# PatrickHwang/Explicit-tf2-Recommendation

Measured on AMD Instinct MI355X. Metric: examples/sec fwd+bwd, DeepFM 10M-vocab x16d batch 8192, higher is better.
Workload: dtype f32; 1 GPU; DeepFM fwd+bwd, 26 categorical fields, 10M-vocab x 16d, batch 8192 (BASELINE.json metric); vocab=10000000, fields=26, embedding_dims=16, batch_per_gpu=8192, id_distribution=uniform, parallelism=single GPU, global_batch=8192, hipgraph=one graph per 5 steps, 32 resident batches

## Files before the change

### explicit-tf2-recommendation_amd/csrc/colsort.hip

```cpp
#include "common.h"

namespace {

constexpr uint32_t PADW = 0xFFFFFFFFu;

struct ColSortArgs {
  int64_t B; int F; int64_t V; int key_bits; int pos_bits; int passes; int digit_bits;
  int32_t* perm;
  int64_t* col_uid;
  int32_t* col_seg;
  int32_t* col_nu;
  int* bad;
  int32_t* dloc;
};

constexpr int CS_T = 1024, CS_W = CS_T / 64, CS_DB = 10, CS_BINS = 1 << CS_DB;
constexpr int CS_BKB = 13, CS_NBK = 1 << CS_BKB, CS_BIG = 32, CS_PROBE = 16;
static_assert(CS_BINS == CS_T, "the count scan gives every thread one digit");

#ifdef REC_SORT_STAMPS
__device__ unsigned long long g_sort_stamps[256 * 16];
#define SSTAMP(k) do { if (threadIdx.x == 0) g_sort_stamps[blockIdx.x * 16 + (k)] = wall_clock64(); } while (0)
#else
#define SSTAMP(k) do {} while (0)
#endif

constexpr int SORT_MAX_COLS = 256;
struct SortCols {
  const int64_t* p[SORT_MAX_COLS];
};

static inline void colsort_digits(int key_bits, int* passes, int* digit_bits) {
  const int p = (key_bits + CS_DB - 1) / CS_DB;
  *passes = p;
  *digit_bits = (key_bits + p - 1) / p;
}

template <int KPT>
__global__ __launch_bounds__(CS_T, 4) void colsort_kernel(SortCols cols, const int64_t* __restrict__ col_lo, ColSortArgs a) {
  extern __shared__ __attribute__((aligned(16))) uint32_t sml[];
  constexpr int NW = CS_T * KPT;
  uint32_t* words = sml;
  uint32_t* cnt = sml + NW;
  uint32_t* wtot = cnt + CS_W * CS_BINS;
  const int tid = threadIdx.x, lane = tid & 63, wave = tid >> 6;
  const int f = blockIdx.x;
  const int64_t B = a.B;
  const int64_t lo = col_lo[f];
  const int pb = a.pos_bits;
  const uint32_t pmask = (1u << pb) - 1u;
  uint32_t* wcnt = cnt + wave * CS_BINS;
  const unsigned long long lt = (1ull << lane) - 1ull;
  SSTAMP(0);
  uint32_t w[KPT];
  bool bad = false;
  const int64_t* col = cols.p[f];
#pragma unroll
  for (int r = 0; r < KPT; ++r) {
    const int e = wave * (64 * KPT) + r * 64 + lane;
    w[r] = PADW;
    if (e < B) {
      const int64_t id = col[e];
      int64_t key = id - lo;
      if (key < 0 || key >= (int64_t(1) << a.key_bits) || (uint64_t)id >= (uint64_t)a.V) {
        bad = true;
        key = key < 0 ? 0 : (int64_t(1) << a.key_bits) - 1;
      }
      w[r] = ((uint32_t)key << pb) | (uint32_t)e;
    }
  }
  if (bad && a.bad) *a.bad = 1;
  SSTAMP(1);
  const int wbits = a.key_bits + pb;
  const int bsh = wbits > CS_BKB ? wbits - CS_BKB : 0;
  uint32_t* bk = cnt;
  static_assert(CS_NBK == 8 * CS_T && CS_NBK <= CS_W * CS_BINS, "8 buckets per thread, inside the counters");
#pragma unroll
  for (int i = 0; i < 2; ++i) reinterpret_cast<uint4*>(bk)[i * CS_T + tid] = make_uint4(0u, 0u, 0u, 0u);
  int hot = 0;
#pragma unroll
  for (int r = 0; r < KPT; ++r) {
    const bool real = wave * (64 * KPT) + r * 64 + lane < B;
    const uint32_t b0 = __shfl(w[r] >> bsh, 0, 64);
    hot |= __popcll(__ballot(real && (w[r] >> bsh) == b0)) > CS_PROBE;
  }
  bool fast = !__syncthreads_or(hot);
  if (fast) {
#pragma unroll
    for (int r = 0; r < KPT; ++r)
      if (wave * (64 * KPT) + r * 64 + lane < B) atomicAdd(&bk[w[r] >> bsh], 1u);
    __syncthreads();
    const uint4 q0 = reinterpret_cast<const uint4*>(bk)[2 * tid], q1 = reinterpret_cast<const uint4*>(bk)[2 * tid + 1];
    uint32_t c[8] = {q0.x, q0.y, q0.z, q0.w, q1.x, q1.y, q1.z, q1.w};
    uint32_t run = 0, mx = 0;
#pragma unroll
    for (int q = 0; q < 8; ++q) {
      run += c[q];
      mx = max(mx, c[q]);
    }
    uint32_t incl = run;
#pragma unroll
    for (int o = 1; o < 64; o <<= 1) {
      const uint32_t t = __shfl_up(incl, o, 64);
      if (lane >= o) incl += t;
    }
    if (lane == 63) wtot[wave] = incl;
    __syncthreads();
    uint32_t base = incl - run;
#pragma unroll
    for (int q = 0; q < CS_W; ++q)
      if (q < wave) base += wtot[q];
#pragma unroll
    for (int q = 0; q < 8; ++q) {
      const uint32_t n = c[q];
      c[q] = base;
      base += n;
    }
    reinterpret_cast<uint4*>(bk)[2 * tid] = make_uint4(c[0], c[1], c[2], c[3]);
    reinterpret_cast<uint4*>(bk)[2 * tid + 1] = make_uint4(c[4], c[5], c[6], c[7]);
    fast = !__syncthreads_or(mx > (uint32_t)CS_BIG);
  }
  SSTAMP(2);
  if (fast) {
#pragma unroll
    for (int r = 0; r < KPT; ++r) {
      const int e = wave * (64 * KPT) + r * 64 + lane;
      if (e < B) words[atomicAdd(&bk[w[r] >> bsh], 1u)] = w[r];
      else words[e] = PADW;
    }
    __syncthreads();
    SSTAMP(3);
    uint32_t dst[KPT];
#pragma unroll
    for (int r = 0; r < KPT; ++r) {
      const int e = wave * (64 * KPT) + r * 64 + lane;
      dst[r] = (uint32_t)e;
      if (e < B) {
        const uint32_t b = w[r] >> bsh;
        const uint32_t end = bk[b];
        uint32_t j = b > 0 ? bk[b - 1] : 0u, rk = j;
        for (; j < end; ++j) rk += words[j] < w[r] ? 1u : 0u;
        dst[r] = rk;
      }
    }
    __syncthreads();
#pragma unroll
    for (int r = 0; r < KPT; ++r) words[dst[r]] = w[r];
    __syncthreads();
    SSTAMP(4);
  }
  for (int pass = 0; pass < (fast ? 0 : a.passes); ++pass) {
    const int shift = pb + pass * a.digit_bits;
    const int nb = min(a.digit_bits, a.key_bits - pass * a.digit_bits);
    const uint32_t dmask = (1u << nb) - 1u;
    if (pass > 0) {
#pragma unroll
      for (int r = 0; r < KPT; ++r) w[r] = words[wave * (64 * KPT) + r * 64 + lane];
    }
#pragma unroll
    for (int i = 0; i < CS_BINS / 256; ++i) reinterpret_cast<uint4*>(wcnt)[i * 64 + lane] = make_uint4(0u, 0u, 0u, 0u);
    uint32_t below[KPT];
#pragma unroll
    for (int c0 = 0; c0 < KPT; c0 += 8) {
      unsigned long long m[8];
#pragma unroll
      for (int r = 0; r < 8; ++r) m[r] = ~0ull;
      for (int b = 0; b < nb; ++b) {
#pragma unroll
        for (int r = 0; r < 8; ++r) {
          const uint32_t s = (uint32_t)__builtin_amdgcn_sbfe((int)w[c0 + r], shift + b, 1);
          const unsigned long long bal = __ballot(s != 0u);
          m[r] &= ~(bal ^ (((unsigned long long)s << 32) | s));
        }
      }
      uint32_t old[8];
      int lead[8];
#pragma unroll
      for (int r = 0; r < 8; ++r) {
        lead[r] = __ffsll((long long)m[r]) - 1;
        below[c0 + r] = (uint32_t)__popcll(m[r] & lt);
        old[r] = 0u;
        if (below[c0 + r] == 0u) old[r] = atomicAdd(&wcnt[(w[c0 + r] >> shift) & dmask], (uint32_t)__popcll(m[r]));
      }
#pragma unroll
      for (int r = 0; r < 8; ++r) below[c0 + r] += (uint32_t)__shfl((int)old[r], lead[r], 64);
    }
    __syncthreads();
    {
      uint32_t c[CS_W];
      uint32_t run = 0;
#pragma unroll
      for (int q = 0; q < CS_W; ++q) {
        c[q] = cnt[q * CS_BINS + tid];
        run += c[q];
      }
      uint32_t incl = run;
#pragma unroll
      for (int o = 1; o < 64; o <<= 1) {
        const uint32_t v = __shfl_up(incl, o, 64);
        if (lane >= o) incl += v;
      }
      if (lane == 63) wtot[wave] = incl;
      __syncthreads();
      uint32_t base = incl - run;
#pragma unroll
      for (int q = 0; q < CS_W; ++q)
        if (q < wave) base += wtot[q];
#pragma unroll
      for (int q = 0; q < CS_W; ++q) {
        cnt[q * CS_BINS + tid] = base;
        base += c[q];
      }
    }
    __syncthreads();
#pragma unroll
    for (int r = 0; r < KPT; ++r) words[wcnt[(w[r] >> shift) & dmask] + below[r]] = w[r];
    __syncthreads();
    SSTAMP(2 + pass);
  }
  const int s0 = tid * KPT;
  uint32_t v[KPT];
  bool hd[KPT];
  int heads = 0;
  uint32_t prev = s0 > 0 ? words[s0 - 1] : PADW;
#pragma unroll
  for (int r = 0; r < KPT; ++r) {
    const int sp = s0 + r;
    v[r] = words[sp];
    const uint32_t pk = (r == 0 ? prev : v[r - 1]) >> pb;
    hd[r] = sp < B && (sp == 0 || (v[r] >> pb) != pk);
    heads += hd[r] ? 1 : 0;
  }
  int incl = heads;
#pragma unroll
  for (int o = 1; o < 64; o <<= 1) {
    const int t = __shfl_up(incl, o, 64);
    if (lane >= o) incl += t;
  }
  if (lane == 63) wtot[wave] = (uint32_t)incl;
  __syncthreads();
  int woff = 0, all = 0;
  for (int q = 0; q < CS_W; ++q) {
    const int c = (int)wtot[q];
    if (q < wave) woff += c;
    all += c;
  }
  int rank = woff + incl - heads;
  SSTAMP(7);
  static_assert(2 * sizeof(unsigned short) * NW <= sizeof(uint32_t) * CS_W * CS_BINS, "the staging fits the counters");
  uint32_t* st_uq = words;
  unsigned short* st_sg = reinterpret_cast<unsigned short*>(cnt);
  unsigned short* st_dl = st_sg + NW;
  int32_t* permf = a.perm + (int64_t)f * B;
  if ((B & 7) == 0 && KPT == 8) {
    if (s0 < B) {
      int4 p0 = make_int4((int)(v[0] & pmask), (int)(v[1] & pmask), (int)(v[2] & pmask), (int)(v[3] & pmask));
      int4 p1 = make_int4((int)(v[4 % KPT] & pmask), (int)(v[5 % KPT] & pmask), (int)(v[6 % KPT] & pmask), (int)(v[7 % KPT] & pmask));
      *reinterpret_cast<int4*>(permf + s0) = p0;
      *reinterpret_cast<int4*>(permf + s0 + 4) = p1;
    }
  } else {
#pragma unroll
    for (int r = 0; r < KPT; ++r)
      if (s0 + r < B) permf[s0 + r] = (int32_t)(v[r] & pmask);
  }
#pragma unroll
  for (int r = 0; r < KPT; ++r) {
    const int sp = s0 + r;
    if (sp < B) {
      if (hd[r]) {
        st_uq[rank] = v[r] >> pb;
        st_sg[rank] = (unsigned short)sp;
        ++rank;
      }
      st_dl[v[r] & pmask] = (unsigned short)(hd[r] ? (rank - 1) : ((rank - 1) | 0x8000));
    }
  }
  __syncthreads();
#pragma unroll
  for (int r = 0; r < KPT; ++r) {
    const int i = r * CS_T + tid;
    if (i < B) {
      if (a.dloc) {
        const uint32_t d = st_dl[i];
        a.dloc[(int64_t)f * B + i] = (int32_t)((d & 0x7FFFu) | ((d & 0x8000u) << 16));
      }
      if (i < all) {
        a.col_uid[(int64_t)f * B + i] = lo + (int64_t)st_uq[i];
        a.col_seg[(int64_t)f * (B + 1) + i] = (int32_t)st_sg[i];
      } else {
        a.col_seg[(int64_t)f * (B + 1) + i] = (int32_t)B;
      }
    }
  }
  if (tid == 0) a.col_seg[(int64_t)f * (B + 1) + B] = (int32_t)B;
  if (tid == 0) a.col_nu[f] = all;
  SSTAMP(8);
#ifdef REC_SORT_STAMPS
  asm volatile("s_waitcnt vmcnt(0)" ::: "memory");
  SSTAMP(9);
  if (threadIdx.x == 1023) g_sort_stamps[blockIdx.x * 16 + 10] = wall_clock64();
  if (threadIdx.x == 512) g_sort_stamps[blockIdx.x * 16 + 11] = wall_clock64();
#endif
}

static int colsort_widths(int64_t B, int64_t max_key, int* key_bits, int* pos_bits) {
  if (B <= 0 || max_key < 0) return REC_E_ARG;
  if (B > 16384) return REC_E_UNSUPPORTED;
  int pbits = 1, kbits = 1;
  while ((int64_t(1) << pbits) < B) ++pbits;
  while ((int64_t(1) << kbits) <= max_key) ++kbits;
  if (kbits + pbits > 32) return REC_E_UNSUPPORTED;
  if ((((uint64_t)max_key << pbits) | (uint64_t)(B - 1)) >= 0xFFFFFFFFull) return REC_E_UNSUPPORTED;
  *key_bits = kbits;
  *pos_bits = pbits;
  return REC_OK;
}
}

#ifdef REC_SORT_STAMPS
extern "C" int rec_debug_sort_stamps(unsigned long long* host_out) {
  return (int)hipMemcpyFromSymbol(host_out, HIP_SYMBOL(g_sort_stamps), sizeof(unsigned long long) * 256 * 16);
}
#endif
extern "C" size_t rec_colsort_workspace_bytes(int64_t B, int F) {
  if (B <= 0 || F <= 0) return 0;
  return 256;
}

extern "C" int rec_colsort_digits(int64_t B, int64_t max_key, int* passes, int* digit_bits) {
  if (!passes || !digit_bits) return REC_E_ARG;
  int key_bits = 0, pos_bits = 0;
  const int rc = colsort_widths(B, max_key, &key_bits, &pos_bits);
  if (rc != REC_OK) return rc;
  colsort_digits(key_bits, passes, digit_bits);
  return REC_OK;
}

static int colsort_plan(const int64_t* const* cols_host, int F, int64_t B, int64_t V, const int64_t* col_lo,
                        int64_t max_key, int32_t* perm, int64_t* col_uid, int32_t* col_seg, int32_t* col_nu,
                        int32_t* dloc, int* bad_flag, void* workspace, void* stream) {
  if (!cols_host || !col_lo || !perm || !col_uid || !col_seg || !col_nu || !workspace || F <= 0 || B <= 0 || V <= 0 ||
      max_key < 0)
    return REC_E_ARG;
  if (F > SORT_MAX_COLS) return REC_E_UNSUPPORTED;
  int key_bits = 0, pos_bits = 0;
  const int rc = colsort_widths(B, max_key, &key_bits, &pos_bits);
  if (rc != REC_OK) return rc;
  int passes = 0, digit_bits = 0;
  colsort_digits(key_bits, &passes, &digit_bits);
  SortCols cp;
  for (int f = 0; f < F; ++f) {
    if (!cols_host[f]) return REC_E_ARG;
    cp.p[f] = cols_host[f];
  }
  ColSortArgs a{B, F, V, key_bits, pos_bits, passes, digit_bits, perm, col_uid, col_seg, col_nu, bad_flag, dloc};
  hipStream_t st = as_stream(stream);
  const int kpt = B <= 8192 ? 8 : 16;
  const size_t lds = sizeof(uint32_t) * ((size_t)CS_T * kpt + CS_W * CS_BINS + CS_W);
  const hipError_t e = kpt == 8 ? rec_allow_lds<colsort_kernel<8>>(lds) : rec_allow_lds<colsort_kernel<16>>(lds);
  if (e != hipSuccess) return (int)e;
  if (kpt == 8)
    hipLaunchKernelGGL(colsort_kernel<8>, dim3(F), dim3(CS_T), lds, st, cp, col_lo, a);
  else
    hipLaunchKernelGGL(colsort_kernel<16>, dim3(F), dim3(CS_T), lds, st, cp, col_lo, a);
  REC_LAUNCH_CHECK();
  return REC_OK;
}

extern "C" int rec_colsort_plan_i64(const int64_t* const* cols_host, int F, int64_t B, int64_t V, const int64_t* col_lo,
                                    int64_t max_key, int32_t* perm, int64_t* col_uid, int32_t* col_seg, int32_t* col_nu,
                                    int* bad_flag, void* workspace, void* stream) {
  return colsort_plan(cols_host, F, B, V, col_lo, max_key, perm, col_uid, col_seg, col_nu, nullptr, bad_flag, workspace,
                      stream);
}

extern "C" int rec_colsort_plan_dest_i64(const int64_t* const* cols_host, int F, int64_t B, int64_t V,
                                         const int64_t* col_lo, int64_t max_key, int32_t* perm, int64_t* col_uid,
                                         int32_t* col_seg, int32_t* col_nu, int32_t* dloc, int* bad_flag, void* workspace,
                                         void* stream) {
  if (!dloc) return REC_E_ARG;
  return colsort_plan(cols_host, F, B, V, col_lo, max_key, perm, col_uid, col_seg, col_nu, dloc, bad_flag, workspace,
                      stream);
}
```

### include/mi355rec.h

```cpp
#ifndef MI355REC_H
#define MI355REC_H

#include <stdint.h>
#include <stddef.h>

#ifdef __cplusplus
extern "C" {
#endif

#define REC_OK 0
#define REC_E_ARG (-1)
#define REC_E_UNSUPPORTED (-2)
#define REC_E_WORKSPACE (-3)

#define REC_MAX_COLS 128

#define REC_AFM_MAX_F 64
#define REC_AFM_MAX_E 64
#define REC_AFM_MAX_A 16
#define REC_AUTOINT_MAX_F 64
#define REC_AUTOINT_MAX_E 64
#define REC_FIBINET_MAX_F 32
#define REC_FIBINET_MAX_E 64
#define REC_FIBINET_MAX_C 64
#define REC_CIN_MAX_F 64
#define REC_CIN_MAX_E 64
#define REC_CIN_MAX_L 8
#define REC_CIN_MAX_H 256
#define REC_FIELD_CONV_MAX_F 64
#define REC_FIELD_CONV_MAX_E 64
#define REC_FIELD_CONV_MAX_L 3
#define REC_FIELD_CONV_MAX_C 16
#define REC_FIELD_CONV_MAX_KW 8
#define REC_FIELD_CONV_BWD_GRID 1024
#define REC_FGCNN_MAX_PW 8
#define REC_MASKNET_MAX_F 64
#define REC_MASKNET_MAX_E 64
#define REC_MASKNET_MAX_D 512
#define REC_MASKNET_MAX_P 512
#define REC_MASKNET_MAX_O 128
#define REC_MASKNET_MAX_R 4

enum { REC_ACT_NONE = 0, REC_ACT_RELU = 1, REC_ACT_SIGMOID = 2, REC_ACT_TANH = 3 };

enum {
  REC_EPI_NONE = 0,
  REC_EPI_BIAS = 1,
  REC_EPI_BIAS_RELU = 2,
  REC_EPI_BIAS_SIGMOID = 3,
  REC_EPI_BIAS_TANH = 4,
  REC_EPI_CROSS = 5,
  REC_EPI_ADD = 6
};

int rec_version(void);

int rec_index_pack_i64(const int64_t* const* cols_host, int F, int64_t rows, int64_t* X, int64_t ldx,
                       int64_t col0, void* stream);

int rec_block_copy(const void* const* srcs_host, int n, int64_t bytes_each, void* out, void* stream);
int rec_auc_hist_update_f32(const float* prob, const float* label, int64_t n, const float* thresholds, int n_thresholds,
                            int64_t* hist, const float* loss_steps, int n_steps, double* loss_acc, void* stream);

int rec_emb_gather_f32(const float* table, int64_t V, int E, int64_t ld, const int64_t* idx, int64_t n,
                       float* out, int* oob_flag, void* stream);

int rec_emb_fm_fwd_f32(const float* embed, int64_t ld_e, const float* w, int64_t ld_w, const float* bias,
                       int64_t V, int E, const int64_t* idx, int64_t B, int F, float* z, float* prob,
                       float* emb_out, float* sumvec, int* oob_flag, void* stream);

int rec_emb_fm_bwd_vals_f32(const float* embed, int64_t ld_e, int64_t V, int E, const int64_t* idx, int64_t B,
                            int F, const float* gz, const float* sumvec, const float* emb_rows,
                            const float* extra, float* dvals, void* stream);

size_t rec_dedup_workspace_bytes(int64_t n);
int rec_dedup_plan_i64(const int64_t* ids, int64_t n, int64_t V, int64_t* uniq_ids, int32_t* seg_start,
                       int32_t* perm, int64_t* n_uniq, void* workspace, size_t workspace_bytes,
                       void* stream);
int rec_dedup_plan_sorted_lists_i64(const int64_t* ids, int64_t n, const int64_t* list_counts, int n_lists,
                                    int64_t V, int64_t* uniq_ids, int32_t* seg_start, int32_t* perm,
                                    int64_t* n_uniq, void* workspace, size_t workspace_bytes, void* stream);
size_t rec_segment_sum_workspace_bytes(int64_t n, int E);
int rec_segment_sum_f32(const float* vals, int E, const int32_t* perm, const int32_t* seg_start, int64_t n,
                        int32_t row_div, float* out, float* workspace, void* stream);

int rec_gemm_f32(int transA, int transB, int64_t M, int64_t N, int64_t K, const float* A, int64_t lda,
                 const float* B, int64_t ldb, float* C, int64_t ldc, int epilogue, const float* bias,
                 const float* e0, int64_t lde0, const float* e1, int64_t lde1, int split_k,
                 float* workspace, float* aux, void* stream);

int rec_crossnet_mat_bwd_elem_f32(const float* g, const float* x0, const float* u, float* h, float* gx0,
                                  int accumulate, int64_t n, void* stream);

int rec_act_fwd_f32(int act, const float* x, const float* x2, float* y, int64_t n, void* stream);
int rec_act_bwd_f32(int act, const float* post, const float* dpost, float* dpre, int64_t n, void* stream);
size_t rec_colsum_workspace_bytes(int64_t M, int64_t N);
int rec_colsum_f32(const float* X, int64_t M, int64_t N, int64_t ldx, float* out, float* workspace, void* stream);
int rec_colsum_fused_f32(const float* X, int64_t M, int64_t N, int64_t ldx, float* out, float* workspace, int* counters,
                         void* stream);
int rec_axpby_f32(float a, const float* x, float b, float* y, int64_t n, void* stream);
int rec_copy_cols_f32(const float* src, int64_t lds, float* dst, int64_t ldd, int64_t rows, int64_t w,
                      void* stream);

int rec_crossnet_vec_fwd_f32(const float* x0, int64_t B, int D, int L, const float* w, const float* b,
                             float* y, float* xs, void* stream);
size_t rec_crossnet_vec_bwd_workspace_bytes(int64_t B, int D, int L);
int rec_crossnet_vec_bwd_f32(const float* x0, int64_t B, int D, int L, const float* w, const float* xs,
                             const float* gy, float* gx0, float* dw, float* db, void* workspace,
                             void* stream);

int rec_cosine_fwd_f32(const float* u, const float* i, int64_t B, int d, float* out, void* stream);
int rec_cosine_bwd_f32(const float* u, const float* i, int64_t B, int d, const float* gout, float* gu,
                       float* gi, void* stream);

int rec_bce_fwd_bwd_f32(const float* y, const float* p, int64_t n, float* loss, float* dp, float* dz,
                        void* stream);

int rec_adam_dense_f32(float* var, float* m, float* v, const float* g, int64_t n, int64_t t, float lr,
                       float b1, float b2, float eps, void* stream);
float rec_adam_lr_t_f32(float lr, float b1, float b2, int64_t t);
int rec_adam_dense_multi_f32(int n_tensors, float* const* var, float* const* m, float* const* v, const float* const* g,
                             const int64_t* numel, const float* lr_t_dev, float b1, float b2, float eps, void* stream);
int rec_adam_sparse_keras_f32(float* var, int64_t ld, float* m, float* v, int64_t V, int E,
                              const int64_t* uniq_ids, const float* g_rows, const int64_t* n_uniq, int64_t cap,
                              float* side, int64_t t, float lr, float b1, float b2, float eps, void* stream);
int rec_adam_sparse_keras_pair_f32(float* fused, int64_t ld, float* m_e, float* v_e, float* m_w, float* v_w, int64_t V,
                                   int E, const int64_t* uniq_ids, const float* g_e_rows, const float* g_w_rows,
                                   const int64_t* n_uniq, int64_t cap, float* side_e, float* side_w, int64_t t,
                                   float lr, float b1, float b2, float eps, void* stream);

int rec_adam_rows_f32(float* var, int64_t ld, float* m, float* v, int64_t V, int E, const int64_t* uniq_ids,
                      const float* g_rows, const int64_t* n_uniq, int64_t cap, int64_t t, float lr,
                      float b1, float b2, float eps, void* stream);

size_t rec_l2_rows_workspace_bytes(int64_t n, int E);
int rec_l2_rows_f32(const float* table, int64_t ld, int64_t V, int E, const int64_t* uniq_ids, const int64_t* n_uniq,
                    int64_t n, float factor, float* rows_out, float* loss, float* workspace, void* stream);

int rec_l2_normalize_rows_f32(const float* x, int64_t n, int d, int64_t ld_in, float* y, int64_t ld_out, void* stream);
size_t rec_topk_l2_workspace_bytes(int64_t nq, int64_t n, int k);
int rec_topk_l2_f32(const float* queries, int64_t nq, int d, int64_t ldq, const float* items, int64_t n, int64_t ldi,
                    int k, int64_t* out_idx, float* out_dist, void* workspace, size_t workspace_bytes, void* stream);

size_t rec_shard_bucketize_workspace_bytes(int64_t n, int n_shard);
int rec_shard_bucketize_i64(const int64_t* ids, int64_t n, int64_t rows_per_shard, int n_shard,
                            int64_t* perm, int64_t* send_counts, int64_t* local_ids, int* oob_flag,
                            void* workspace, size_t workspace_bytes, void* stream);
int rec_colsort_shard_map_i64(const int32_t* perm, const int64_t* col_uid, const int32_t* col_seg,
                              const int32_t* col_nu, int64_t B, int F, int64_t rows_per_shard, int n_shard,
                              int64_t* uid_local, int64_t* uidx, int64_t* send_counts, int64_t* n_uniq,
                              int* oob_flag, void* stream);
int rec_colsort_shard_map_fixed_i64(const int32_t* perm, const int64_t* col_uid, const int32_t* col_seg,
                                    const int32_t* col_nu, int64_t B, int F, int64_t rows_per_shard, int n_shard,
                                    int64_t cap, int64_t* msg, int64_t* uidx, int32_t* slot_map, int64_t* n_uniq,
                                    int* oob_flag, void* stream);
int rec_shard_slab_map_uslot_i64(const int64_t* uniq_ids, const int64_t* n_uniq, const int32_t* seg_start,
                                 const int32_t* perm, int64_t n, int64_t rows_per_shard, int n_shard, int64_t cap,
                                 int64_t* msg, int64_t* slot, int64_t* uslot, int* oob_flag, void* stream);
int rec_emb_gather_lists_f32(const float* table, int64_t V, int E, int64_t ld, const int64_t* msg, int n_lists,
                             int64_t cap, float* out, int* oob_flag, void* stream);
int rec_dedup_plan_sorted_slabs_i64(const int64_t* msg, int n_lists, int64_t cap, int64_t V, int64_t* uniq_ids,
                                    int32_t* seg_start, int32_t* perm, int64_t* n_uniq, void* workspace,
                                    size_t workspace_bytes, void* stream);
int rec_permute_rows_f32(const float* in, const int64_t* perm, int64_t n, int E, int scatter, float* out,
                         void* stream);

size_t rec_deepfm_fused_workspace_bytes(int64_t B, int F);

size_t rec_colsort_workspace_bytes(int64_t B, int F);
int rec_colsort_digits(int64_t B, int64_t max_key, int* passes, int* digit_bits);
int rec_colsort_plan_i64(const int64_t* const* cols_host, int F, int64_t B, int64_t V, const int64_t* col_lo,
                         int64_t max_key, int32_t* perm, int64_t* col_uid, int32_t* col_seg, int32_t* col_nu,
                         int* bad_flag, void* workspace, void* stream);
int rec_colsort_plan_dest_i64(const int64_t* const* cols_host, int F, int64_t B, int64_t V, const int64_t* col_lo,
                              int64_t max_key, int32_t* perm, int64_t* col_uid, int32_t* col_seg, int32_t* col_nu,
                              int32_t* dloc, int* bad_flag, void* workspace, void* stream);

int rec_deepfm_k0t_f32(const float* K0, int F, float* K0T, void* stream);
int rec_deepfm_fused3_main_f32(const float* table, int64_t ld, int64_t V, const int64_t* const* cols_host, int F,
                               int64_t B, const float* const* weights, const float* label, float* gz, float* vals,
                               float* prob, int* oob_flag, void* workspace, const int32_t* dloc, const int32_t* col_nu,
                               float* g_embed_rows, int64_t* step_dev, const float* lr_table, int64_t n_table,
                               float* lr_t_dev, void* stream);

typedef struct rec_deepfm_lazy_adam {
  float* table; int64_t ld, V;
  float *m_e, *v_e, *m_w, *v_w; int64_t ld_state, ld_wstate;
  const float* lr_t_dev; float b1, b2, eps;
  int32_t* last; const int64_t* step_dev;
} rec_deepfm_lazy_adam;
int rec_deepfm_fused_post_f32(int F, int64_t B, const float* gz, const float* vals, float* const* grads, float* loss,
                              void* workspace, const int32_t* perm, const int64_t* col_uid, const int32_t* col_seg,
                              const int32_t* col_nu, int64_t* uniq_ids, float* g_embed_rows, float* g_w_rows,
                              int64_t* n_uniq, const int32_t* slot_map, int direct, const rec_deepfm_lazy_adam* adam,
                              void* stream);
int rec_adam_keras_catchup_f32(const int64_t* col_uid, const int32_t* col_nu, int64_t B, int F, float* table, int64_t ld,
                               int64_t V, float* m_e, float* v_e, int64_t ld_state, float* m_w, float* v_w,
                               int64_t ld_wstate, const int32_t* last, const int64_t* step_dev, const float* lr_table,
                               int64_t n_table, float b1, float b2, float eps, void* stream);
int rec_adam_keras_flush_f32(float* table, int64_t ld, int64_t V, float* m_e, float* v_e, int64_t ld_state, float* m_w,
                             float* v_w, int64_t ld_wstate, int32_t* last, const int64_t* step_dev, const float* lr_table,
                             int64_t n_table, float b1, float b2, float eps, void* stream);

size_t rec_dssm_fused_workspace_bytes(int64_t B, int E, int F_u, int F_i);
int rec_dssm_fused_main_f32(const float* u_table, int64_t u_ld, int64_t u_V, const int64_t* u_ids, int F_u,
                            const float* i_table, int64_t i_ld, int64_t i_V, const int64_t* i_ids, int F_i, int E,
                            int h1, int h2, int d_out, int64_t B, const float* const* weights, const float* label,
                            float* u_vals, float* i_vals, float* user_emb, float* item_emb, float* score, int* oob_flag,
                            void* workspace, size_t workspace_bytes, int64_t* step_dev, const float* lr_table,
                            int64_t n_table, float* lr_t_dev, void* stream);
int rec_dssm_fused_post_f32(int64_t B, int E, int F_u, int F_i, const void* workspace, size_t workspace_bytes,
                            float* const* grads, float* loss, const float* u_vals, const int32_t* u_perm,
                            const int32_t* u_seg, const int64_t* u_uniq, const int64_t* u_n_uniq, float* u_rows,
                            const float* i_vals, const int32_t* i_perm, const int32_t* i_seg, const int64_t* i_uniq,
                            const int64_t* i_n_uniq, float* i_rows, float* const* adam, int64_t u_ld, int64_t u_V,
                            int64_t i_ld, int64_t i_V, const float* lr_t_dev, float b1, float b2, float eps,
                            void* stream);

enum { REC_DACT_NONE = 0, REC_DACT_RELU = 1, REC_DACT_SIGMOID = 2, REC_DACT_TANH = 3,
       REC_DACT_DICE = 4,
       REC_DACT_PRELU = 5 };
int rec_din_prepare_f32(const float* W1, const float* b1, int D, int H, float* Wcat, float* Wkd, float* bext,
                        void* stream);
int rec_din_prepare_bwd_f32(const float* gWcat, const float* gWkd, int D, int H, float* gW1, void* stream);
int rec_din_attn_fwd_f32(const float* embed, int64_t ld, int64_t V, int E, int C, const int64_t* series, int64_t B,
                         int T, const float* Mext, const float* Wkd, int H, int act, const float* alpha,
                         const float* mean, const float* var, const float* w2, const float* b2,
                         int64_t padding_index, int mask_valid, float* scores, float* pooled, int* oob_flag,
                         void* stream);
int rec_din_attn_bwd_f32(const float* embed, int64_t ld, int64_t V, int E, int C, const int64_t* series, int64_t B,
                         int T, const float* Mext, const float* Wkd, int H, int act, const float* alpha,
                         const float* mean, const float* var, const float* w2, const float* b2,
                         int64_t padding_index, int mask_valid, const float* scores, const float* gpooled,
                         float* gkeys, float* gMext, float* gw2p, float* galphap, float* gb2p, void* stream);

int rec_feat_act_fwd_f32(int kind, const float* x, const float* alpha, const float* mean, const float* var, float* y,
                         int64_t M, int N, void* stream);
int rec_feat_act_bwd_f32(int kind, const float* x, const float* gy, const float* alpha, const float* mean,
                         const float* var, float* gx, float* ga_elem, int64_t M, int N, void* stream);
int rec_layernorm_fwd_f32(const float* x, const float* gamma, const float* beta, int64_t M, int N, float* y,
                          float* xhat, float* rstd, void* stream);
int rec_layernorm_bwd_f32(const float* gy, const float* xhat, const float* rstd, const float* gamma, int64_t M, int N,
                          float* gx, float* gg_elem, void* stream);
int rec_softmax_fwd_f32(const float* x, int64_t M, int N, float* y, void* stream);
int rec_softmax_bwd_f32(const float* y, const float* gy, int64_t M, int N, float* gx, void* stream);


int rec_emb_ipn_fwd_f32(const float* table, int64_t V, int E, int64_t ld, const int64_t* X, int64_t B, int F,
                        float* out, int64_t ld_out, int* oob_flag, void* stream);
int rec_emb_ipn_bwd_vals_f32(const float* out, int64_t ld_out, const float* g, int64_t ld_g, int64_t B, int F, int E,
                             float* vals, void* stream);

int rec_emb_bi_fwd_f32(const float* table, int64_t V, int E, int64_t ld, const int64_t* X, int64_t B, int F, float* out,
                       int64_t ld_out, float* sumvec, int* oob_flag, void* stream);
int rec_emb_bi_bwd_vals_f32(const float* table, int64_t V, int E, int64_t ld, const int64_t* X, int64_t B, int F,
                            const float* g, int64_t ld_g, const float* sumvec, float* vals, void* stream);

int rec_ip_attn_fwd_f32(const float* embed, int64_t ld, int64_t V, int E, int C, const int64_t* series, int64_t B, int T,
                        const float* q, int64_t ld_q, int64_t padding_index, float* scores, float* pooled,
                        int64_t ld_pooled, int* oob_flag, void* stream);
int rec_ip_attn_bwd_f32(const float* embed, int64_t ld, int64_t V, int E, int C, const int64_t* series, int64_t B, int T,
                        const float* q, int64_t ld_q, int64_t padding_index, const float* scores, const float* gpooled,
                        int64_t ld_gpooled, float* gkeys, float* gq, void* stream);

int rec_ffm_fwd_f32(const float* v, int64_t ld_v, const float* w, int64_t ld_w, const float* bias, int64_t V, int E,
                    const int64_t* X, int64_t B, int F, float* z, float* prob, int* oob_flag, void* stream);
int rec_ffm_bwd_rows_f32(const float* v, int64_t ld_v, int64_t V, int E, const int64_t* X, int64_t B, int F,
                         const float* gz, const int32_t* perm, const int32_t* seg_start, const int64_t* n_uniq,
                         float* g_rows, void* stream);

size_t rec_batchnorm_workspace_bytes(int64_t B, int N);
int rec_batchnorm_fwd_f32(const float* x, int64_t ld_x, int64_t B, int N, const float* gamma, const float* beta,
                          float eps, float momentum, int training, float* moving_mean, float* moving_var, float* y,
                          float* xhat, float* rstd, void* workspace, void* stream);
int rec_batchnorm_bwd_f32(const float* g, const float* xhat, const float* rstd, int64_t B, int N, const float* gamma,
                          int training, float* gx, float* ggamma, float* gbeta, void* workspace, void* stream);

size_t rec_cin_workspace_bytes(int64_t B, int F, int E, int L, const int* H_host);
int rec_cin_fwd_f32(const float* x0, int64_t B, int F, int E, int L, const int* H_host, const float* const* W_host,
                    float* states, float* cin_part, void* stream);
int rec_cin_bwd_f32(const float* x0, const float* states, const float* g, int64_t B, int F, int E, int L,
                    const int* H_host, const float* const* W_host, float* dx0, float* const* dW_host, void* workspace,
                    size_t workspace_bytes, void* stream);

size_t rec_fibinet_workspace_bytes(int64_t B, int F, int E, int mid, int type);
int rec_fibinet_fwd_f32(const float* x_emb, const float* x_cont, const float* S0, const float* S1, const float* W,
                        int64_t B, int F, int E, int C, int mid, int type, float* dnn_in, float* A, float* H1,
                        void* stream);
int rec_fibinet_bwd_f32(const float* x_emb, const float* g, const float* A, const float* H1, const float* S0,
                        const float* S1, const float* W, int64_t B, int F, int E, int C, int mid, int type,
                        float* dx_emb, float* dW, float* dS0, float* dS1, void* workspace, size_t workspace_bytes,
                        void* stream);

size_t rec_autoint_workspace_bytes(int64_t B, int F, int E, int H, int C, int res);
int rec_autoint_fwd_f32(const float* x, const float* x_cont, const float* cemb, const float* Wq, const float* Wk,
                        const float* Wv, const float* Wres, int64_t B, int F, int E, int H, int C, int res, int scaling,
                        float* y, float* o, float* stats, void* workspace, size_t workspace_bytes, void* stream);
int rec_autoint_bwd_f32(const float* x, const float* x_cont, const float* cemb, const float* Wq, const float* Wk,
                        const float* Wv, const float* Wres, const float* y, const float* dy, const float* stats,
                        int64_t B, int F, int E, int H, int C, int res, int scaling, float* dx, float* dWq, float* dWk,
                        float* dWv, float* dWres, float* dcemb, void* workspace, size_t workspace_bytes, void* stream);

size_t rec_afm_workspace_bytes(int64_t B, int F, int E, int A);
int rec_emb_afm_fwd_f32(const float* table, int64_t V, int E, int64_t ld, const int64_t* X, int64_t B, int F, int A,
                        const float* Wa, const float* ba, const float* hv, const float* bh, float* o, float* stats,
                        float* rows, int* oob_flag, void* stream);
int rec_emb_afm_bwd_f32(const float* table, int64_t V, int E, int64_t ld, const int64_t* X, int64_t B, int F, int A,
                        const float* Wa, const float* ba, const float* hv, const float* bh, const float* o,
                        const float* stats, const float* rows, const float* dout, float* vals, float* dWa, float* dba,
                        float* dhv, float* dbh, void* workspace, size_t workspace_bytes, void* stream);

size_t rec_ccpm_workspace_bytes(int64_t B, int F, int E, int L, const int* filters_host, const int* kernel_width_host,
                                const int* pool_k_host);
int rec_emb_ccpm_fwd_f32(const float* table, int64_t V, int E, int64_t ld, const int64_t* X, int64_t B, int F, int L,
                         const int* filters_host, const int* kernel_width_host, const int* pool_k_host,
                         const float* params, float* out, float* rows, int* oob_flag, void* stream);
int rec_emb_ccpm_bwd_f32(const float* table, int64_t V, int E, int64_t ld, const int64_t* X, int64_t B, int F, int L,
                         const int* filters_host, const int* kernel_width_host, const int* pool_k_host,
                         const float* params, const float* rows, const float* dout, float* vals, float* dparams,
                         void* workspace, size_t workspace_bytes, void* stream);

size_t rec_fgcnn_workspace_bytes(int64_t B, int F, int E, int L, const int* filters_host, const int* kernel_width_host,
                                 const int* pooling_width_host);
int rec_emb_fgcnn_fwd_f32(const float* table, int64_t V, int E, int64_t ld, const int64_t* X, int64_t B, int F, int L,
                          const int* filters_host, const int* kernel_width_host, const int* pooling_width_host,
                          const float* params, float* rows_out, float* const* pooled_out_host_ptrs, int* oob_flag,
                          void* stream);
int rec_emb_fgcnn_bwd_f32(int E, int64_t B, int F, int L, const int* filters_host, const int* kernel_width_host,
                          const int* pooling_width_host, const float* params, const float* rows,
                          const float* const* dpooled_host_ptrs, const float* drows_direct, float* vals, float* dparams,
                          void* workspace, size_t workspace_bytes, void* stream);

size_t rec_masknet_ln_workspace_bytes(int64_t B, int F, int E);
int rec_emb_masknet_ln_fwd_f32(const float* table, int64_t V, int E, int64_t ld, const int64_t* X, const float* values,
                               int64_t B, int F, int Fk, const float* gamma, const float* beta, float* x_emb,
                               float* x_norm, float* stats, int* oob_flag, void* stream);
int rec_emb_masknet_ln_bwd_f32(const float* x_emb, const float* stats, const float* values, const float* gamma,
                               const float* dx_norm, const float* dx_emb, int64_t B, int F, int Fk, int E, float* vals,
                               float* dgamma, float* dbeta, void* workspace, size_t workspace_bytes, void* stream);
size_t rec_masknet_block_workspace_bytes(int64_t B, int D, int P, int O, int R);
int rec_mask_block_fwd_f32(const float* x_emb, const float* v, const float* W1, const float* b1, const float* W2,
                           const float* b2, const float* W3, const float* b3, const float* gamma, const float* beta,
                           int64_t B, int D, int P, int O, int R, float* y, float* h, float* m, float* xhat, float* rstd,
                           void* stream);
int rec_mask_block_bwd_f32(const float* x_emb, const float* v, const float* W1, const float* W2, const float* W3,
                           const float* gamma, const float* y, const float* h, const float* m, const float* xhat,
                           const float* rstd, const float* dy, int64_t B, int D, int P, int O, int R, float* dv,
                           float* dx_emb, int accumulate, float* dW1, float* db1, float* dW2, float* db2, float* dW3,
                           float* db3, float* dgamma, float* dbeta, void* workspace, size_t workspace_bytes,
                           void* stream);

int rec_emb_contextnet_in_fwd_f32(const float* table, int64_t V, int E, int64_t ld, const int64_t* X,
                                  const float* values, int64_t B, int F, int Fk, float* x, int* oob_flag, void* stream);
int rec_emb_contextnet_in_bwd_f32(const float* values, const float* dx, int64_t B, int F, int Fk, int E, float* vals,
                                  void* stream);
size_t rec_contextnet_block_workspace_bytes(int64_t B, int F, int E, int R, int pointwise);
int rec_contextnet_block_fwd_f32(const float* x, const float* Wa, const float* ba, const float* Wb, const float* bb,
                                 const float* W1, const float* W2, const float* gamma, const float* beta, int64_t B,
                                 int F, int E, int R, int pointwise, float* y, float* h, float* m, float* xhat,
                                 float* rstd, float* a, void* stream);
int rec_contextnet_block_bwd_f32(const float* x, const float* Wa, const float* Wb, const float* W1, const float* W2,
                                 const float* gamma, const float* h, const float* m, const float* xhat,
                                 const float* rstd, const float* a, const float* dy, int64_t B, int F, int E, int R,
                                 int pointwise, float* dx, float* dWa, float* dba, float* dWb, float* dbb, float* dW1,
                                 float* dW2, float* dgamma, float* dbeta, void* workspace, size_t workspace_bytes,
                                 void* stream);

size_t rec_emb_fibinetplus_in_workspace_bytes(int64_t B, int F, int Fk, int E);
int rec_emb_fibinetplus_in_fwd_f32(const float* table, int64_t V, int E, int64_t ld, const int64_t* X,
                                   const float* values, const float* gamma_bn, const float* beta_bn,
                                   const float* gamma_ln, const float* beta_ln, int64_t B, int F, int Fk, int training,
                                   float* moving_mean, float* moving_var, float* x, float* xhat, float* rstd_bn,
                                   float* rstd_ln, int* oob_flag, void* workspace, size_t workspace_bytes, void* stream);
int rec_emb_fibinetplus_in_bwd_f32(const float* dx, const float* values, const float* xhat, const float* rstd_bn,
                                   const float* rstd_ln, const float* gamma_bn, const float* gamma_ln, int64_t B, int F,
                                   int Fk, int E, int training, float* vals, float* dgamma_bn, float* dbeta_bn,
                                   float* dgamma_ln, float* dbeta_ln, void* workspace, size_t workspace_bytes,
                                   void* stream);
size_t rec_fibinetplus_block_workspace_bytes(int64_t B, int F, int E, int G, int mid, int O, int type);
int rec_fibinetplus_block_fwd_f32(const float* x, const float* W, const float* Wr, const float* br,
                                  const float* gamma_q, const float* beta_q, const float* S0, const float* b0,
                                  const float* gamma0, const float* beta0, const float* S1, const float* b1,
                                  const float* gamma1, const float* beta1, int64_t B, int F, int E, int G, int mid, int O,
                                  int type, float* out, float* p, float* xhat_q, float* s, float* xhat0, float* h,
                                  float* xhat1, float* rstd, void* stream);
int rec_fibinetplus_block_bwd_f32(const float* x, const float* W, const float* Wr, const float* gamma_q, const float* S0,
                                  const float* gamma0, const float* beta0, const float* S1, const float* gamma1,
                                  const float* beta1, const float* p, const float* xhat_q, const float* s,
                                  const float* xhat0, const float* h, const float* xhat1, const float* rstd,
                                  const float* dout, int64_t B, int F, int E, int G, int mid, int O, int type, float* dx,
                                  float* dW, float* dWr, float* dbr, float* dgamma_q, float* dbeta_q, float* dS0,
                                  float* db0, float* dgamma0, float* dbeta0, float* dS1, float* db1, float* dgamma1,
                                  float* dbeta1, void* workspace, size_t workspace_bytes, void* stream);

size_t rec_mmoe_workspace_bytes(int64_t B, int D, int n, int T, int H1, int O, int H2, int O2);
int rec_mmoe_fwd_f32(const float* x, const float* W1, const float* b1, const float* We2, const float* be2,
                     const float* Wg2, const float* bg2, const float* Wt1, const float* bt1, const float* Wt2,
                     const float* bt2, const float* Wt3, const float* bt3, int64_t B, int D, int n, int T, int H1, int O,
                     int H2, int O2, int gate_softmax_passes, int ctcvr, float* out, float* h, float* e, float* z,
                     float* g, float* a1, float* a2, float* p, void* stream);
int rec_mmoe_bwd_f32(const float* x, const float* W1, const float* We2, const float* Wg2, const float* Wt1,
                     const float* Wt2, const float* Wt3, const float* h, const float* e, const float* z, const float* g,
                     const float* a1, const float* a2, const float* p, const float* dout, int64_t B, int D, int n, int T,
                     int H1, int O, int H2, int O2, int gate_softmax_passes, int ctcvr, float* dx, float* dW1,
                     float* db1, float* dWe2, float* dbe2, float* dWg2, float* dbg2, float* dWt1, float* dbt1,
                     float* dWt2, float* dbt2, float* dWt3, float* dbt3, void* workspace, size_t workspace_bytes,
                     void* stream);

#ifdef __cplusplus
}
#endif
#endif
```

Before: 243.3 million examples/s.

## Add LDS bitmap-rank path to per-column sort for small key ranges

Adds a path to the column sort kernel for the case where each field's key range fits in an LDS bitmap. Each key sets a bit, and a popcount prefix scan over the bitmap gives its unique rank and position directly, replacing the bucket and radix passes. Duplicate keys are counted per word and resolved through a small slow list with a linear comparison. If the slow list overflows its cap, or keys exceed max_key, the kernel falls back to the existing path, at the cost of more code, more LDS zeroing and extra branches.

```diff
diff --git a/explicit-tf2-recommendation_amd/csrc/colsort.hip b/explicit-tf2-recommendation_amd/csrc/colsort.hip
--- a/explicit-tf2-recommendation_amd/csrc/colsort.hip
+++ b/explicit-tf2-recommendation_amd/csrc/colsort.hip
@@ -11,18 +11,31 @@
   int32_t* col_seg;
   int32_t* col_nu;
   int* bad;
+  int64_t max_key;
+  int bm_words;
   int32_t* dloc;
 };
 
 constexpr int CS_T = 1024, CS_W = CS_T / 64, CS_DB = 10, CS_BINS = 1 << CS_DB;
 constexpr int CS_BKB = 13, CS_NBK = 1 << CS_BKB, CS_BIG = 32, CS_PROBE = 16;
 static_assert(CS_BINS == CS_T, "the count scan gives every thread one digit");
+constexpr int CS_BM_WORDS = 13 * CS_T, CS_BM_CAP = 512, CS_BM_PPT = 7;
+constexpr int CS_BM_XC = CS_BM_WORDS, CS_BM_PU = CS_BM_XC + CS_BM_WORDS / 2, CS_BM_LIST = CS_BM_PU + CS_BM_WORDS / 4,
+              CS_BM_REC = CS_BM_LIST + CS_BM_CAP, CS_BM_WTOT = CS_BM_REC + CS_BM_CAP, CS_BM_END = CS_BM_WTOT + CS_W;
+static_assert(CS_BM_PPT * CS_T * 2 >= CS_BM_WORDS && CS_BM_WORDS % 8 == 0, "the scan covers the bitmap, 16-byte zeroing");
+static_assert(CS_BM_END <= CS_T * 8 + CS_W * CS_BINS, "the bitmap path fits the LDS of the other paths at 8 words per thread");
+static_assert(CS_BM_REC % 2 == 0 && CS_BM_XC % 4 == 0, "8-byte records, 16-byte zeroing of xc");
+static_assert(CS_T * 8 * 2 <= CS_BM_PU, "the staging leaves pu, list and records alone");
 
 #ifdef REC_SORT_STAMPS
 __device__ unsigned long long g_sort_stamps[256 * 16];
 #define SSTAMP(k) do { if (threadIdx.x == 0) g_sort_stamps[blockIdx.x * 16 + (k)] = wall_clock64(); } while (0)
+#define SSTAMP_END() do { SSTAMP(8); asm volatile("s_waitcnt vmcnt(0)" ::: "memory"); SSTAMP(9); \
+    if (threadIdx.x == 1023) g_sort_stamps[blockIdx.x * 16 + 10] = wall_clock64(); \
+    if (threadIdx.x == 512) g_sort_stamps[blockIdx.x * 16 + 11] = wall_clock64(); } while (0)
 #else
 #define SSTAMP(k) do {} while (0)
+#define SSTAMP_END() do {} while (0)
 #endif
 
 constexpr int SORT_MAX_COLS = 256;
@@ -54,18 +67,30 @@
   SSTAMP(0);
   uint32_t w[KPT];
   bool bad = false;
+  const int nw = KPT == 8 ? a.bm_words : 0;
+  int hot = 0;
   const int64_t* col = cols.p[f];
+  int64_t id[KPT];
+#pragma unroll
+  for (int r = 0; r < KPT; ++r) {
+    const int e = wave * (64 * KPT) + r * 64 + lane;
+    id[r] = e < B ? col[e] : lo;
+  }
+  uint32_t* bm = sml;
+  uint32_t* xc32 = sml + CS_BM_XC;
+  for (int i = tid; i < (nw + 3) / 4; i += CS_T) reinterpret_cast<uint4*>(bm)[i] = make_uint4(0u, 0u, 0u, 0u);
+  for (int i = tid; i < (nw + 7) / 8; i += CS_T) reinterpret_cast<uint4*>(xc32)[i] = make_uint4(0u, 0u, 0u, 0u);
 #pragma unroll
   for (int r = 0; r < KPT; ++r) {
     const int e = wave * (64 * KPT) + r * 64 + lane;
     w[r] = PADW;
     if (e < B) {
-      const int64_t id = col[e];
-      int64_t key = id - lo;
-      if (key < 0 || key >= (int64_t(1) << a.key_bits) || (uint64_t)id >= (uint64_t)a.V) {
+      int64_t key = id[r] - lo;
+      if (key < 0 || key >= (int64_t(1) << a.key_bits) || (uint64_t)id[r] >= (uint64_t)a.V) {
         bad = true;
         key = key < 0 ? 0 : (int64_t(1) << a.key_bits) - 1;
       }
+      if (nw && key > a.max_key) hot = 1;
       w[r] = ((uint32_t)key << pb) | (uint32_t)e;
     }
   }
@@ -75,9 +100,10 @@
   const int bsh = wbits > CS_BKB ? wbits - CS_BKB : 0;
   uint32_t* bk = cnt;
   static_assert(CS_NBK == 8 * CS_T && CS_NBK <= CS_W * CS_BINS, "8 buckets per thread, inside the counters");
-#pragma unroll
-  for (int i = 0; i < 2; ++i) reinterpret_cast<uint4*>(bk)[i * CS_T + tid] = make_uint4(0u, 0u, 0u, 0u);
-  int hot = 0;
+  if (!nw) {
+#pragma unroll
+    for (int i = 0; i < 2; ++i) reinterpret_cast<uint4*>(bk)[i * CS_T + tid] = make_uint4(0u, 0u, 0u, 0u);
+  }
 #pragma unroll
   for (int r = 0; r < KPT; ++r) {
     const bool real = wave * (64 * KPT) + r * 64 + lane < B;
@@ -85,6 +111,220 @@
     hot |= __popcll(__ballot(real && (w[r] >> bsh) == b0)) > CS_PROBE;
   }
   bool fast = !__syncthreads_or(hot);
+  if (KPT == 8 && nw && fast) {
+    uint32_t was[KPT];
+#pragma unroll
+    for (int r = 0; r < KPT; ++r) {
+      const uint32_t key = w[r] >> pb, bit = 1u << (key & 31u);
+      was[r] = 0u;
+      if (wave * (64 * KPT) + r * 64 + lane < B) was[r] = atomicOr(&bm[key >> 5], bit) & bit;
+    }
+#pragma unroll
+    for (int r = 0; r < KPT; ++r) {
+      const uint32_t wd = w[r] >> (pb + 5);
+      if (was[r]) atomicAdd(&xc32[wd >> 1], (wd & 1u) ? 0x10000u : 1u);
+    }
+    __syncthreads();
+    SSTAMP(12);
+    const int npairs = (nw + 1) >> 1;
+    const uint2* bm2 = reinterpret_cast<const uint2*>(bm);
+    uint2 bw[CS_BM_PPT];
+    uint32_t xw[CS_BM_PPT];
+#pragma unroll
+    for (int i = 0; i < CS_BM_PPT; ++i) {
+      const int p = min(tid * CS_BM_PPT + i, npairs - 1);
+      bw[i] = bm2[p];
+      xw[i] = xc32[p];
+    }
+    uint32_t accA = 0, accS = 0;
+#pragma unroll
+    for (int i = 0; i < CS_BM_PPT; ++i) {
+      if (tid * CS_BM_PPT + i >= npairs) {
+        bw[i] = make_uint2(0u, 0u);
+        xw[i] = 0u;
+      }
+      const uint32_t x0 = xw[i] & 0xFFFFu, x1 = xw[i] >> 16;
+      const uint32_t c0 = (uint32_t)__popc(bw[i].x), c1 = (uint32_t)__popc(bw[i].y);
+      accA += c0 + c1 + ((x0 + x1) << 16);
+      accS += (x0 ? 1u + ((c0 + x0) << 16) : 0u) + (x1 ? 1u + ((c1 + x1) << 16) : 0u);
+    }
+    uint32_t inA = accA, inS = accS;
+#pragma unroll
+    for (int o = 1; o < 64; o <<= 1) {
+      const uint32_t tA = __shfl_up(inA, o, 64), tS = __shfl_up(inS, o, 64);
+      if (lane >= o) {
+        inA += tA;
+        inS += tS;
+      }
+    }
+    uint32_t* wtotS = sml + CS_BM_WTOT;
+    if (lane == 63) {
+      wtot[wave] = inA;
+      wtotS[wave] = inS;
+    }
+    __syncthreads();
+    uint32_t A = inA - accA, S = inS - accS, allA = 0, allS = 0;
+#pragma unroll
+    for (int q = 0; q < CS_W; ++q) {
+      const uint32_t tA = wtot[q], tS = wtotS[q];
+      if (q < wave) {
+        A += tA;
+        S += tS;
+      }
+      allA += tA;
+      allS += tS;
+    }
+    const uint32_t nslow = allS >> 16;
+    if (nslow <= (uint32_t)CS_BM_CAP) {
+      const int all = (int)(allA & 0xFFFFu);
+      unsigned short* pu = reinterpret_cast<unsigned short*>(sml + CS_BM_PU);
+      uint32_t* list = sml + CS_BM_LIST;
+      uint2* rec = reinterpret_cast<uint2*>(sml + CS_BM_REC);
+#pragma unroll
+      for (int i = 0; i < CS_BM_PPT; ++i) {
+        const int p = tid * CS_BM_PPT + i;
+        if (p < npairs) {
+          const uint32_t xs[2] = {xw[i] & 0xFFFFu, xw[i] >> 16};
+          const uint32_t cs[2] = {(uint32_t)__popc(bw[i].x), (uint32_t)__popc(bw[i].y)};
+          uint32_t o[2];
+          pu[p] = (unsigned short)(A & 0xFFFFu);
+#pragma unroll
+          for (int h = 0; h < 2; ++h) {
+            o[h] = A >> 16;
+            if (xs[h]) {
+              o[h] = 0x8000u | (S & 0xFFFFu);
+              rec[S & 0xFFFFu] = make_uint2((A >> 16) | (S & 0xFFFF0000u), S >> 16);
+              S += 1u + ((cs[h] + xs[h]) << 16);
+            }
+            A += cs[h] + (xs[h] << 16);
+          }
+          xc32[p] = o[0] | (o[1] << 16);
+        }
+      }
+      __syncthreads();
+      SSTAMP(13);
+      const unsigned short* xc16 = reinterpret_cast<const unsigned short*>(xc32);
+      uint32_t xv[KPT], run[KPT], pos[KPT];
+#pragma unroll
+      for (int c0 = 0; c0 < KPT; c0 += 4) {
+        uint32_t b0[4], b1[4];
+#pragma unroll
+        for (int q = 0; q < 4; ++q) {
+          const int r = c0 + q;
+          const bool real = wave * (64 * KPT) + r * 64 + lane < B;
+          const uint32_t wd = real ? w[r] >> (pb + 5) : 0u;
+          const uint2 t = bm2[wd >> 1];
+          b0[q] = t.x;
+          b1[q] = t.y;
+          xv[r] = real ? (uint32_t)xc16[wd] : 0u;
+          run[r] = pu[wd >> 1];
+        }
+#pragma unroll
+        for (int q = 0; q < 4; ++q) {
+          const int r = c0 + q;
+          pos[r] = 0u;
+          if (xv[r] & 0x8000u) pos[r] = atomicAdd(&rec[xv[r] & 0x7FFFu].y, 1u);
+        }
+#pragma unroll
+        for (int q = 0; q < 4; ++q) {
+          const int r = c0 + q;
+          if (xv[r] & 0x8000u) {
+            list[pos[r]] = w[r];
+          } else {
+            const uint32_t key = w[r] >> pb, wd = key >> 5, below = (1u << (key & 31u)) - 1u;
+            const uint32_t odd = 0u - (wd & 1u);
+            run[r] += (uint32_t)__popc(b0[q] & odd) + (uint32_t)__popc(((b1[q] & odd) | (b0[q] & ~odd)) & below);
+            pos[r] = run[r] + xv[r];
+          }
+        }
+      }
+      __syncthreads();
+      uint32_t s_w = 0, s_pos = 0, s_run = 0;
+      bool s_hd = false;
+      if ((uint32_t)tid < nslow) {
+        s_w = list[tid];
+        const uint32_t key = s_w >> pb, wd = key >> 5, below = (1u << (key & 31u)) - 1u;
+        const uint2 b = bm2[wd >> 1];
+        const uint32_t odd = 0u - (wd & 1u), bx = b.x, by = b.y;
+        const uint32_t base = pu[wd >> 1] + (uint32_t)__popc(bx & odd);
+        const uint2 t = rec[xc16[wd] & 0x7FFFu];
+        const uint32_t sb = t.x >> 16, end = min(t.y, (uint32_t)CS_BM_CAP);
+        uint32_t v[4], c = 0, same = 0;
+#pragma unroll
+        for (int q = 0; q < 4; ++q) v[q] = list[min(sb + q, (uint32_t)CS_BM_CAP - 1u)];
+#pragma unroll
+        for (int q = 0; q < 4; ++q) {
+          const bool lt = sb + q < end && v[q] < s_w;
+          c += lt ? 1u : 0u;
+          same += (lt && (v[q] >> pb) == key) ? 1u : 0u;
+        }
+        for (uint32_t j = sb + 4; j < end; ++j) {
+          const uint32_t u = list[j];
+          c += u < s_w ? 1u : 0u;
+          same += (u < s_w && (u >> pb) == key) ? 1u : 0u;
+        }
+        s_run = base + (uint32_t)__popc(((by & odd) | (bx & ~odd)) & below);
+        s_pos = base + (t.x & 0xFFFFu) + c;
+        s_hd = same == 0u;
+      }
+      __syncthreads();
+      uint32_t* st_uq = sml;
+      unsigned short* st_sg = reinterpret_cast<unsigned short*>(sml + NW);
+      unsigned short* st_pm = st_sg + NW;
+      int32_t* permf = a.perm + (int64_t)f * B;
+#pragma unroll
+      for (int r = 0; r < KPT; ++r) {
+        const int e = wave * (64 * KPT) + r * 64 + lane;
+        if (e < B && !(xv[r] & 0x8000u)) {
+          st_pm[pos[r]] = (unsigned short)e;
+          st_uq[run[r]] = w[r] >> pb;
+          st_sg[run[r]] = (unsigned short)pos[r];
+          if (a.dloc) a.dloc[(int64_t)f * B + e] = (int32_t)run[r];
+        }
+      }
+      if ((uint32_t)tid < nslow) {
+        const uint32_t e = s_w & pmask;
+        st_pm[s_pos] = (unsigned short)e;
+        if (s_hd) {
+          st_uq[s_run] = s_w >> pb;
+          st_sg[s_run] = (unsigned short)s_pos;
+        }
+        if (a.dloc) a.dloc[(int64_t)f * B + e] = (int32_t)(s_run | (s_hd ? 0u : 0x80000000u));
+      }
+      __syncthreads();
+      SSTAMP(14);
+      if ((B & 7) == 0) {
+        if (tid * 8 < B) {
+          const uint4 q = reinterpret_cast<const uint4*>(st_pm)[tid];
+          *reinterpret_cast<int4*>(permf + tid * 8) = make_int4((int)(q.x & 0xFFFFu), (int)(q.x >> 16), (int)(q.y & 0xFFFFu), (int)(q.y >> 16));
+          *reinterpret_cast<int4*>(permf + tid * 8 + 4) = make_int4((int)(q.z & 0xFFFFu), (int)(q.z >> 16), (int)(q.w & 0xFFFFu), (int)(q.w >> 16));
+        }
+      } else {
+#pragma unroll
+        for (int r = 0; r < KPT; ++r)
+          if (r * CS_T + tid < B) permf[r * CS_T + tid] = (int32_t)st_pm[r * CS_T + tid];
+      }
+#pragma unroll
+      for (int r = 0; r < KPT; ++r) {
+        const int i = r * CS_T + tid;
+        if (i < B) {
+          if (i < all) {
+            a.col_uid[(int64_t)f * B + i] = lo + (int64_t)st_uq[i];
+            a.col_seg[(int64_t)f * (B + 1) + i] = (int32_t)st_sg[i];
+          } else {
+            a.col_seg[(int64_t)f * (B + 1) + i] = (int32_t)B;
+          }
+        }
+      }
+      if (tid == 0) a.col_seg[(int64_t)f * (B + 1) + B] = (int32_t)B;
+      if (tid == 0) a.col_nu[f] = all;
+      SSTAMP_END();
+      return;
+    }
+#pragma unroll
+    for (int i = 0; i < 2; ++i) reinterpret_cast<uint4*>(bk)[i * CS_T + tid] = make_uint4(0u, 0u, 0u, 0u);
+    __syncthreads();
+  }
   if (fast) {
 #pragma unroll
     for (int r = 0; r < KPT; ++r)
@@ -295,13 +535,7 @@
   }
   if (tid == 0) a.col_seg[(int64_t)f * (B + 1) + B] = (int32_t)B;
   if (tid == 0) a.col_nu[f] = all;
-  SSTAMP(8);
-#ifdef REC_SORT_STAMPS
-  asm volatile("s_waitcnt vmcnt(0)" ::: "memory");
-  SSTAMP(9);
-  if (threadIdx.x == 1023) g_sort_stamps[blockIdx.x * 16 + 10] = wall_clock64();
-  if (threadIdx.x == 512) g_sort_stamps[blockIdx.x * 16 + 11] = wall_clock64();
-#endif
+  SSTAMP_END();
 }
 
 static int colsort_widths(int64_t B, int64_t max_key, int* key_bits, int* pos_bits) {
@@ -326,6 +560,21 @@
 extern "C" size_t rec_colsort_workspace_bytes(int64_t B, int F) {
   if (B <= 0 || F <= 0) return 0;
   return 256;
+}
+
+static inline int colsort_bitmap_words(int64_t B, int64_t max_key) {
+  const int64_t nw = (max_key + 32) / 32;
+  return B <= 8192 && nw <= CS_BM_WORDS ? (int)nw : 0;
+}
+
+extern "C" int rec_colsort_bitmap_limits(int64_t B, int64_t max_key, int* words, int* slow_cap) {
+  if (!words || !slow_cap) return REC_E_ARG;
+  int key_bits = 0, pos_bits = 0;
+  const int rc = colsort_widths(B, max_key, &key_bits, &pos_bits);
+  if (rc != REC_OK) return rc;
+  *words = colsort_bitmap_words(B, max_key);
+  *slow_cap = CS_BM_CAP;
+  return REC_OK;
 }
 
 extern "C" int rec_colsort_digits(int64_t B, int64_t max_key, int* passes, int* digit_bits) {
@@ -354,7 +603,8 @@
     if (!cols_host[f]) return REC_E_ARG;
     cp.p[f] = cols_host[f];
   }
-  ColSortArgs a{B, F, V, key_bits, pos_bits, passes, digit_bits, perm, col_uid, col_seg, col_nu, bad_flag, dloc};
+  ColSortArgs a{B, F, V, key_bits, pos_bits, passes, digit_bits, perm, col_uid, col_seg, col_nu, bad_flag, max_key,
+                colsort_bitmap_words(B, max_key), dloc};
   hipStream_t st = as_stream(stream);
   const int kpt = B <= 8192 ? 8 : 16;
   const size_t lds = sizeof(uint32_t) * ((size_t)CS_T * kpt + CS_W * CS_BINS + CS_W);
diff --git a/include/mi355rec.h b/include/mi355rec.h
--- a/include/mi355rec.h
+++ b/include/mi355rec.h
@@ -169,6 +169,7 @@
 
 size_t rec_colsort_workspace_bytes(int64_t B, int F);
 int rec_colsort_digits(int64_t B, int64_t max_key, int* passes, int* digit_bits);
+int rec_colsort_bitmap_limits(int64_t B, int64_t max_key, int* words, int* slow_cap);
 int rec_colsort_plan_i64(const int64_t* const* cols_host, int F, int64_t B, int64_t V, const int64_t* col_lo,
                          int64_t max_key, int32_t* perm, int64_t* col_uid, int32_t* col_seg, int32_t* col_nu,
                          int* bad_flag, void* workspace, void* stream);
```

New measurement: 250.1 million examples/s, median of 6. +2.8%, better.
